# chengzhag/PanFusion

Hardware: AMD Instinct MI355X
Metric: DDIM denoise steps/sec, 512x1024 pano + 20x512^2 views (higher is better)
Workload: dtype fp16; 1 GPU; cfg2: 512x1024 pano + 20x512^2 views, CFG pair, SD-2-base UNet shapes; views=20, cfg_pair=True, hip_graphs=True, parallelism=single

## Files before the change

### include/panfusion_hip.h

```cpp
#ifndef PANFUSION_HIP_H
#define PANFUSION_HIP_H

#include <stddef.h>
#include <stdint.h>

#ifdef __cplusplus
extern "C" {
#endif

typedef enum { PF_OK = 0, PF_ERR_ARG = 1, PF_ERR_LAUNCH = 2, PF_ERR_UNSUPPORTED = 3 } pf_status;
typedef enum { PF_BF16 = 0, PF_F16 = 1, PF_F32 = 2, PF_U8 = 3 } pf_dtype;

int pf_version(void);
const char* pf_last_error_string(void);


pf_status pf_e2p_grid(const double* host_fov, const double* host_theta, const double* host_phi,
                      int ncam, int eh, int ew, int h, int w,
                      float* map_x, float* map_y, float* lonlat, void* stream);

pf_status pf_p2e_grid(const double* host_fov, const double* host_theta, const double* host_phi,
                      int ncam, int ph, int pw, int h, int w,
                      float* map_u, float* map_v, uint8_t* mask, void* stream);

// ... 182 lines not shown
    int M, N, K;
    int dtype; int mode;
} pf_linear_ws_desc;
enum { PF_LWS_16 = 0, PF_LWS_F32 = 1, PF_LWS_GEGLU = 2, PF_LWS_QKV = 3, PF_LWS_F32_LN = 4, PF_LWS_VT = 5 };
int pf_linear_ws_supported(long M, int N, int K, int mode);
pf_status pf_linear_ws(const pf_linear_ws_desc* desc, void* stream);

pf_status pf_conv_in(const float* x, int n, int cin, int h, int w, const float* wgt, const float* bias,
                     int cout, int wrap, int out_dtype, void* y, void* stream);
pf_status pf_conv_out(const void* x, int dtype, int n, int cin, int h, int w, const float* wgt,
                      const float* bias, int cout, int wrap, float* y, void* stream);
pf_status pf_conv_out_gn(const float* x, int n, int cin, int h, int w, const float* scale, const float* shift, int act,
                         const float* wgt_t, const float* bias, int cout, int wrap, float* y, void* stream);

typedef struct {
    const void* q; const void* k; const void* vt; void* out;
    int dtype;
    int B, H, D;
    int nq, nk;
    int q_ld, k_ld, vt_ld, o_ld;
    long q_bs, k_bs, vt_bs, o_bs;
    float scale;
    const float* bias; long bias_ld;
    const uint8_t* flags; int flags_ld;
    float* lse;
    void* workspace; size_t workspace_bytes;
} pf_attn_desc;

pf_status pf_attention(const pf_attn_desc* desc, void* stream);
size_t pf_attention_workspace_size(const pf_attn_desc* desc);

pf_status pf_attention_wide(const pf_attn_desc* desc, void* stream);


pf_status pf_attention_delta(const void* out, const void* dout, int dtype, int B, int H, int D, long nq,
                             int ld, long bs, float* delta, void* stream);

typedef struct {
    const void* q; const void* k; const void* v; const void* dout;
    const void* qt; const void* kt; const void* dot;
    void* dq; void* dk; void* dv;
    int dtype;
    int B, H, D;
    int nq, nk;
    int q_ld, k_ld, v_ld, do_ld;
    int qt_ld, kt_ld, dot_ld;
    int dq_ld, dk_ld, dv_ld;
    long q_bs, k_bs, v_bs, do_bs, qt_bs, kt_bs, dot_bs, dq_bs, dk_bs, dv_bs;
    float scale;
    const float* bias; long bias_ld;
    const uint8_t* flags; int flags_ld;
    const float* lse; const float* delta;
    void* workspace; size_t workspace_bytes;
} pf_attn_bwd_desc;

size_t pf_attention_bwd_workspace_size(const pf_attn_bwd_desc* desc);
pf_status pf_attention_bwd(const pf_attn_bwd_desc* desc, void* stream);

int pf_layernorm_bwd_parts(long rows);
pf_status pf_layernorm_bwd(const void* x, const float* pe, long pe_rows, int dtype, long rows, int C,
                           const float* gamma, float eps, const float* dy, const float* dres, float* dx,
                           float* partials, void* stream);

size_t pf_groupnorm_bwd_workspace_size(int n_img, int hw, int groups);
pf_status pf_groupnorm_bwd(const void* x0, int c0, const void* x1, int c1, int dtype, int n_img, int hw, int groups,
                           float eps, const float* gamma, const float* scale, const float* shift, int act,
// ... 44 lines not shown
```

### panfusion_amd/_lib.py

```python
import ctypes as C
import os

_HERE = os.path.dirname(os.path.abspath(__file__))
LIB_PATH = os.environ.get("PF_HIP_LIB") or os.path.join(_HERE, "libpanfusion_hip.so")

PF_OK = 0
PF_BF16, PF_F16, PF_F32, PF_U8 = 0, 1, 2, 3

c_void_p, c_int, c_long, c_float, c_size_t = C.c_void_p, C.c_int, C.c_long, C.c_float, C.c_size_t
c_dp = C.POINTER(C.c_double)


class ConvDesc(C.Structure):
    _fields_ = [
        ("a0", c_void_p), ("a1", c_void_p), ("c0", c_int), ("c1", c_int),
        ("a0_ld", c_int), ("a1_ld", c_int),
        ("n_img", c_int), ("h_in", c_int), ("w_in", c_int), ("h_out", c_int), ("w_out", c_int),
        ("ksize", c_int), ("stride", c_int), ("pad", c_int), ("upsample", c_int),
        ("w", c_void_p), ("n_out", c_int),
        ("bias", c_void_p), ("rowvec", c_void_p), ("rowvec_ld", c_int),
        ("residual", c_void_p), ("res_ld", c_int), ("res_dtype", c_int),
        ("out", c_void_p), ("out_ld", c_int), ("out_dtype", c_int), ("dtype", c_int),
        ("batch", c_int),
        ("a_bstride", c_long), ("w_bstride", c_long), ("out_bstride", c_long), ("res_bstride", c_long),
# ... 3 lines not shown
        ("a_src_dtype", c_int), ("a_scale", c_void_p), ("a_shift", c_void_p),
    ]


class ConvPlan(C.Structure):
    _fields_ = [
        ("kernel", c_int), ("mrep", c_int), ("nrep", c_int), ("block_rows", c_int), ("waves", c_int), ("ring_slots", c_int),
        ("splits", c_int), ("kb_per_split", c_int), ("m_split", c_int), ("tail_splits", c_int), ("tail_kb", c_int),
        ("gn_rows", c_int), ("n_tickets", c_int), ("workspace_bytes", c_size_t),
    ]


class AttnDesc(C.Structure):
    _fields_ = [
        ("q", c_void_p), ("k", c_void_p), ("vt", c_void_p), ("out", c_void_p),
        ("dtype", c_int), ("B", c_int), ("H", c_int), ("D", c_int), ("nq", c_int), ("nk", c_int),
        ("q_ld", c_int), ("k_ld", c_int), ("vt_ld", c_int), ("o_ld", c_int),
        ("q_bs", c_long), ("k_bs", c_long), ("vt_bs", c_long), ("o_bs", c_long),
        ("scale", c_float),
        ("bias", c_void_p), ("bias_ld", c_long), ("flags", c_void_p), ("flags_ld", c_int),
        ("lse", c_void_p),
        ("workspace", c_void_p), ("workspace_bytes", c_size_t),
    ]


class LinearWsDesc(C.Structure):
    _fields_ = [
        ("a", c_void_p), ("a_ld", c_int), ("w", c_void_p), ("bias", c_void_p),
        ("residual", c_void_p), ("res_ld", c_int), ("out", c_void_p), ("out_ld", c_int),
        ("out_vt", c_void_p), ("vt_ld", c_int), ("rows_per_batch", c_int), ("vt_bs", c_long),
        ("ln_gamma", c_void_p), ("ln_beta", c_void_p), ("ln_eps", c_float), ("ln_out", c_void_p), ("ln_ld", c_int),
        ("M", c_int), ("N", c_int), ("K", c_int), ("dtype", c_int), ("mode", c_int),
    ]


class AttnBwdDesc(C.Structure):
    _fields_ = [
        ("q", c_void_p), ("k", c_void_p), ("v", c_void_p), ("dout", c_void_p),
        ("qt", c_void_p), ("kt", c_void_p), ("dot", c_void_p),
        ("dq", c_void_p), ("dk", c_void_p), ("dv", c_void_p),
        ("dtype", c_int), ("B", c_int), ("H", c_int), ("D", c_int), ("nq", c_int), ("nk", c_int),
        ("q_ld", c_int), ("k_ld", c_int), ("v_ld", c_int), ("do_ld", c_int),
        ("qt_ld", c_int), ("kt_ld", c_int), ("dot_ld", c_int),
        ("dq_ld", c_int), ("dk_ld", c_int), ("dv_ld", c_int),
        ("q_bs", c_long), ("k_bs", c_long), ("v_bs", c_long), ("do_bs", c_long), ("qt_bs", c_long), ("kt_bs", c_long),
        ("dot_bs", c_long), ("dq_bs", c_long), ("dk_bs", c_long), ("dv_bs", c_long),
        ("scale", c_float),
        ("bias", c_void_p), ("bias_ld", c_long), ("flags", c_void_p), ("flags_ld", c_int),
        ("lse", c_void_p), ("delta", c_void_p),
        ("workspace", c_void_p), ("workspace_bytes", c_size_t),
    ]


SIGNATURES = {
    "pf_version": (c_int, []),
    "pf_last_error_string": (C.c_char_p, []),
    "pf_e2p_grid": (c_int, [c_dp, c_dp, c_dp, c_int, c_int, c_int, c_int, c_int,
                            c_void_p, c_void_p, c_void_p, c_void_p]),
    "pf_p2e_grid": (c_int, [c_dp, c_dp, c_dp, c_int, c_int, c_int, c_int, c_int,
                            c_void_p, c_void_p, c_void_p, c_void_p]),
    "pf_py360_e2p": (c_int, [c_void_p, c_int, c_int, c_int, c_int, c_dp, c_dp, c_dp, c_dp, c_dp, c_int, c_int, c_int, c_int,
                             c_void_p, c_void_p]),
    "pf_nearest_indices": (c_int, [c_void_p, c_void_p, c_long, c_int, c_int, c_void_p, c_void_p]),
    "pf_remap": (c_int, [c_void_p, c_int, c_int, c_int, c_int, c_int, c_void_p, c_void_p, c_void_p,
                         c_int, c_int, c_int, c_int, c_void_p, c_void_p]),
    "pf_equi_coords": (c_int, [c_int, c_int, c_void_p, c_void_p]),
# ... 32 lines not shown
                                      c_long, c_int, c_int, c_void_p, c_void_p, c_void_p, c_int, C.c_int64, c_void_p]),
    "pf_cfg_dpmpp_step_pair": (c_int, [c_void_p, c_void_p, c_void_p, c_float, c_float, c_float, c_float, c_float,
                                       c_long, c_int, c_int, c_void_p, c_void_p, c_void_p, c_int, C.c_int64,
                                       c_void_p, c_float, c_void_p, c_void_p]),
    "pf_cfg_inpaint_step_pair": (c_int, [c_void_p, c_void_p, c_void_p, c_float, c_float, c_float, c_float, c_float,
                                         c_long, c_int, c_int, c_void_p, c_void_p, c_void_p, c_int, C.c_int64,
                                         c_void_p, c_float, c_void_p, c_void_p, c_void_p, c_void_p, c_float, c_float,
                                         c_int, c_void_p]),
    "pf_noised_start_pair": (c_int, [c_void_p, c_void_p, c_float, c_float, c_long, c_int, c_int, c_void_p, c_void_p, c_void_p,
                                     c_int, C.c_int64, c_void_p]),
    "pf_upsampled_start_pair": (c_int, [c_void_p, c_void_p, c_float, c_float, c_long, c_int, c_int, c_int, c_int, c_int, c_int,
                                        c_int, c_void_p, c_void_p, c_void_p, c_int, C.c_int64, c_void_p]),
    "pf_conv_gemm":(c_int, [C.POINTER(ConvDesc), c_void_p]),
    "pf_conv_gemm_workspace_size": (c_size_t, [C.POINTER(ConvDesc)]),
    "pf_conv_gemm_gn_rows": (c_int, [C.POINTER(ConvDesc)]),
    "pf_conv_gemm_kernel_id": (c_int, [C.POINTER(ConvDesc)]),
    "pf_conv_gemm_plan": (c_int, [C.POINTER(ConvDesc), c_int, C.POINTER(ConvPlan)]),
    "pf_groupnorm_from_partials": (c_int, [c_void_p, c_int, c_int, c_void_p, c_int, c_int, c_int, c_int, c_int, c_float,
                                           c_void_p, c_void_p, c_void_p, c_void_p, c_void_p]),
    "pf_scale_shift_act_pair": (c_int, [c_void_p, c_int, c_void_p, c_int, c_int, c_int, c_void_p, c_void_p, c_int, c_int,
                                        c_void_p, c_void_p, c_void_p]),
    "pf_debug_gemm_profile": (c_int, [c_void_p, c_long]),
    "pf_linear_ws_supported": (c_int, [c_long, c_int, c_int, c_int]),
    "pf_linear_ws": (c_int, [C.POINTER(LinearWsDesc), c_void_p]),
    "pf_conv_in": (c_int, [c_void_p, c_int, c_int, c_int, c_int, c_void_p, c_void_p, c_int, c_int, c_int,
                           c_void_p, c_void_p]),
    "pf_conv_out": (c_int, [c_void_p, c_int, c_int, c_int, c_int, c_int, c_void_p, c_void_p, c_int, c_int,
                            c_void_p, c_void_p]),
    "pf_conv_out_gn": (c_int, [c_void_p, c_int, c_int, c_int, c_int, c_void_p, c_void_p, c_int, c_void_p, c_void_p, c_int, c_int,
                               c_void_p, c_void_p]),
    "pf_attention": (c_int, [C.POINTER(AttnDesc), c_void_p]),
    "pf_attention_workspace_size": (c_size_t, [C.POINTER(AttnDesc)]),
    "pf_attention_wide": (c_int, [C.POINTER(AttnDesc), c_void_p]),
    "pf_attention_delta": (c_int, [c_void_p, c_void_p, c_int, c_int, c_int, c_int, c_long, c_int, c_long, c_void_p, c_void_p]),
    "pf_attention_bwd": (c_int, [C.POINTER(AttnBwdDesc), c_void_p]),
    "pf_attention_bwd_workspace_size": (c_size_t, [C.POINTER(AttnBwdDesc)]),
    "pf_layernorm_bwd_parts": (c_int, [c_long]),
    "pf_layernorm_bwd": (c_int, [c_void_p, c_void_p, c_long, c_int, c_long, c_int, c_void_p, c_float, c_void_p, c_void_p,
                                 c_void_p, c_void_p, c_void_p]),
    "pf_groupnorm_bwd_workspace_size": (c_size_t, [c_int, c_int, c_int]),
    "pf_groupnorm_bwd": (c_int, [c_void_p, c_int, c_void_p, c_int, c_int, c_int, c_int, c_int, c_float, c_void_p, c_void_p,
                                 c_void_p, c_int, c_void_p, c_void_p, c_void_p, c_void_p, c_void_p, c_size_t, c_void_p]),
    "pf_groupnorm_param_grads_workspace_size": (c_size_t, [c_int, c_int, c_int]),
    "pf_groupnorm_param_grads": (c_int, [c_void_p, c_int, c_void_p, c_int, c_int, c_int, c_int, c_void_p, c_void_p, c_void_p, c_void_p,
                                         c_int, c_void_p, c_void_p, c_void_p, c_size_t, c_void_p]),
    "pf_silu_bwd": (c_int, [c_void_p, c_int, c_void_p, c_long, c_void_p, c_void_p]),
    "pf_im2col3": (c_int, [c_void_p, c_int, c_int, c_int, c_int, c_int, c_int, c_void_p, c_void_p]),
    "pf_lora_fold": (c_int, [c_void_p, c_void_p, c_void_p, c_int, c_int, c_int, c_float, c_int, c_void_p, c_long, c_void_p, c_long,
                             c_void_p, c_long, c_void_p, c_long, c_void_p]),
    "pf_weighted_colsum_workspace_size": (c_size_t, [c_long, c_int, c_int]),
    "pf_weighted_colsum": (c_int, [c_void_p, c_int, c_long, c_int, c_long, c_void_p, c_int, c_long, c_void_p, c_float, c_void_p, c_int,
                                   c_void_p, c_void_p, c_size_t, c_void_p]),
    "pf_zero_insert2": (c_int, [c_void_p, c_int, c_int, c_int, c_int, c_int, c_void_p, c_void_p]),
    "pf_sum2x2": (c_int, [c_void_p, c_int, c_int, c_int, c_int, c_void_p, c_void_p]),
    "pf_pad_width_bwd": (c_int, [c_void_p, c_int, c_int, c_int, c_int, c_int, c_void_p, c_void_p]),
    "pf_crop_width_bwd": (c_int, [c_void_p, c_int, c_int, c_int, c_int, c_int, c_void_p, c_void_p]),
    "pf_transpose_tokens": (c_int, [c_void_p, c_int, c_int, c_long, c_int, c_void_p, c_void_p]),
    "pf_geglu_bwd": (c_int, [c_void_p, c_void_p, c_int, c_long, c_int, c_void_p, c_void_p]),
    "pf_colsum_workspace_size": (c_size_t, [c_long, c_int]),
    "pf_colsum": (c_int, [c_void_p, c_int, c_long, c_int, c_long, c_void_p, c_void_p, c_size_t, c_void_p]),
    "pf_amax_f32": (c_int, [c_void_p, c_long, c_void_p, c_int, c_void_p]),
    "pf_pow2_scale": (c_int, [c_void_p, c_void_p]),
    "pf_scale_f32": (c_int, [c_void_p, c_long, c_void_p, c_int, c_int, c_void_p, c_void_p]),
}


# ... 44 lines not shown
```

### panfusion_amd/engine.py

```python
import os
from types import SimpleNamespace as NS

import torch

from . import ops


def default_precision(dtype):
    env = os.environ.get("PF_PRECISION")
    if env in ("mixed", "fast"):
        return env
    return "mixed" if dtype == torch.float16 else "fast"


RAW_PAIR_FUSED = os.environ.get("PF_RAW_PAIR", "1") != "0"
A32 = os.environ.get("PF_A32", "1") != "0"
TAPING = False
VIRTUAL_PAD = os.environ.get("PF_VIRTUAL_PAD", "1") != "0"
EXACT_UP0 = os.environ.get("PF_EXACT_UP0", "1") != "0"
SUBPIXEL_UP = os.environ.get("PF_SUBPIXEL_UP", "1") != "0"
FUSED_HEAD = os.environ.get("PF_FUSED_HEAD", "1") != "0"


def stream_dtype(dtype, precision):
# ... 400 lines not shown
        y = ops.scale_shift_act(x, skip, n, hw, sc, sh, 1, out_dtype=r.dtype)
    rowvec = temb_all[:, r.temb_off:] if temb_all is not None else None
    wp = w + 2 * wrap
    h1 = ops.conv_gemm(y, r.w1, r.cout, n_img=n, h_in=h, w_in=w, ksize=3, pad=1, bias=r.b1, rowvec=rowvec, gn_stats=True,
                       wrap_pad=wrap, out_dtype=torch.float32 if save is not None else None)
    h1 = ops.carry(h1.view(n, h * wp, r.cout), h1)
    sc, sh = ops.groupnorm_scale_shift(h1, None, n, h * wp, r.norm2.groups, r.norm2.eps, r.norm2.g, r.norm2.b)
    if save is not None:
        save.h1, save.sc2, save.sh2 = h1, sc, sh
    y2 = ops.scale_shift_act(h1, None, n, h * wp, sc, sh, 1, out_dtype=r.dtype)
    if split:
        short = _split_shortcut(r, x, n * hw, max_operand_bytes)
    elif r.ws3 is not None:
        if direct:
            short = exact_gemm_f32(x, r.ws3, r.cout, r.dtype, x1=skip, w_in=n * hw, bias=r.bs, out_dtype=r.stream)
        else:
            if pair is None:
                pair = split_operand(x, skip, dtype=r.dtype)
            short = exact_gemm(pair, r.ws3, r.cout, w_in=n * hw, bias=r.bs, out_dtype=r.stream)
    elif r.ws is not None:
        short = ops.conv_gemm(x, r.ws, r.cout, a1=skip, n_img=n, h_in=h, w_in=w, ksize=1, bias=r.bs)
    else:
        short = x.view(n * hw, r.cout)
    out = ops.conv_gemm(y2, r.w2, r.cout, n_img=n, h_in=h, w_in=wp, ksize=3, pad=1, bias=r.b2, residual=short, gn_stats=True,
                        crop=wrap)
    return ops.carry(out.view(n, h, w, r.cout), out)


def text_kv(a, text):
    n, L = text.shape[:2]
    return ops.linear(text.reshape(n * L, -1), a.wk), ops.linear_t(text, a.wv)


def all_transformers(u):
    for blk in [*u.down, u.mid, *u.up]:
        for t in (blk.attns or []):
            yield t


def self_qkv(a, tokens, n, nk):
    fused = ops.linear_qkv(tokens, a.wqkv, n)
    if fused is not None:
        return fused
    qk = ops.linear(tokens, a.wqk)
    vt = ops.linear_vt(tokens, a.wv, n)
    if vt is None:
        vt = ops.linear_t(tokens.view(n, nk, -1), a.wv)
    return qk, vt


def _attend(a, q_src, kv_tokens, n, nq, nk, head_dim, *, self_attn, residual, kv=None, next_ln=None, split=None):
    Cq = a.dim
    vt = None
    if split is not None and self_attn and n == 1:
        from . import sharding
        o = sharding.split_pano_attention(split, a, q_src, nq)
        if next_ln is not None:
            return ops.linear_ln(o.view(n * nq, Cq), a.wo, a.bo, residual, next_ln.g, next_ln.b, next_ln.eps)
        return ops.linear(o.view(n * nq, Cq), a.wo, bias=a.bo, residual=residual)
    if self_attn:
        qk, vt = self_qkv(a, q_src, n, nk)
        q, k, ld = qk, qk[:, Cq:], 2 * Cq
    else:
        q, ld = ops.linear(q_src, a.wq), Cq
        k = kv[0] if kv is not None else ops.linear(kv_tokens, a.wk)
    if kv is not None:
        vt = kv[1]
    elif vt is None:
        vt = ops.linear_t(kv_tokens.view(n, nk, -1), a.wv)
    o = ops.attention(q, k, vt, n, a.heads, head_dim, nq, nk,
                      q_ld=ld, k_ld=(ld if self_attn else Cq), vt_ld=vt.shape[-1],
                      q_bs=nq * ld, k_bs=nk * (ld if self_attn else Cq), vt_bs=vt.shape[1] * vt.shape[2])
    if next_ln is not None:
        return ops.linear_ln(o.view(n * nq, Cq), a.wo, a.bo, residual, next_ln.g, next_ln.b, next_ln.eps)
    return ops.linear(o.view(n * nq, Cq), a.wo, bias=a.bo, residual=residual)


def run_transformer(t, x, text, kv=None, split=None):
    n, h, w, Cc = x.shape
    hw = h * w
    sc, sh = ops.groupnorm_scale_shift(x, None, n, hw, t.norm.groups, t.norm.eps, t.norm.g, t.norm.b)
    if t.w_in3 is not None:
        tok = exact_gemm_f32(x, t.w_in3, Cc, t.dtype, scale=sc, shift=sh, w_in=n * hw, bias=t.b_in, out_dtype=t.stream)
    else:
        y = ops.scale_shift_act(x, None, n, hw, sc, sh, 0)
        tok = ops.linear(y.view(n * hw, Cc), t.w_in, bias=t.b_in)
    dh = t.attn1.dim // t.attn1.heads
    ln = ops.layernorm(tok, t.ln1.g, t.ln1.b, t.ln1.eps, out_dtype=t.dtype)
    tok, ln = _attend(t.attn1, ln, ln, n, hw, hw, dh, self_attn=True, residual=tok, next_ln=t.ln2, split=split)
    if ln is None:
        ln = ops.layernorm(tok, t.ln2.g, t.ln2.b, t.ln2.eps, out_dtype=t.dtype)
    L = text.shape[1]
    tok, ln = _attend(t.attn2, ln, text.reshape(n * L, -1), n, hw, L, dh, self_attn=False, residual=tok, kv=kv, next_ln=t.ln3)
    if ln is None:
        ln = ops.layernorm(tok, t.ln3.g, t.ln3.b, t.ln3.eps, out_dtype=t.dtype)
    g = ops.linear(ln, t.w_ff1, bias=t.b_ff1, geglu=True)
    if t.w_out3 is not None and os.environ.get("PF_FF2_PAIR", "1") != "0":
        pair = ops.linear(g, t.w_ff2, bias=t.b_ff2, residual=tok, split_out=True)
        out = exact_gemm(pair, t.w_out3, Cc, w_in=n * hw, bias=t.b_out, residual=x.view(n * hw, Cc), gn_stats=True)
    elif t.w_out3 is not None:
        tok = ops.linear(g, t.w_ff2, bias=t.b_ff2, residual=tok)
        out = exact_gemm(split_operand(tok, dtype=t.dtype), t.w_out3, Cc, w_in=n * hw, bias=t.b_out, residual=x.view(n * hw, Cc),
                         gn_stats=True)
    else:
        tok = ops.linear(g, t.w_ff2, bias=t.b_ff2, residual=tok)
        out = ops.linear(tok, t.w_out, bias=t.b_out, residual=x.view(n * hw, Cc), gn_stats=True)
    return ops.carry(out.view(n, h, w, Cc), out)


class Branch:

    def __init__(self, u, latent, timestep, text, pano, pad):
        self.u, self.text, self.pad = u, text, (pano and pad)
        n = latent.shape[0]
        feats = ops.timestep_features(timestep, u.t_dim, u.dtype)
        e = ops.linear(feats, u.w_t1, bias=u.b_t1)
        e = ops.linear(ops.silu(e), u.w_t2, bias=u.b_t2)
        self.temb = ops.linear(ops.silu(e), u.w_temb, bias=u.b_temb, out_dtype=torch.float32)
        self.h = ops.conv_in(latent.float(), u.w_conv_in, u.b_conv_in, u.c0, u.stream, wrap=self.pad)
        self.skips = [self.h]
        self.text_kv = {}
        self.text_ready = None
        self.attn_split = None
        self.attn_help = None
        self.split_streams = None
        self.keep = None

    def precompute_text_kv(self):
        key = (self.text.data_ptr(), self.text._version, tuple(self.text.shape), self.text.dtype, str(self.text.device))
        cache = self.u.__dict__.setdefault("text_kv_cache", {})
        hit = cache.get(key)
        if hit is None:
            if len(cache) >= 4:
                victim = next((ck for ck, h in cache.items() if not h.get("pins")), None)
                if victim is not None:
                    cache.pop(victim)
            hit = {id(t): text_kv(t.attn2, self.text) for t in all_transformers(self.u)}
            hit["text"] = self.text
            cache[key] = hit
        self.text_kv = hit

    def _padded(self, t, p):
        return ops.pad_width(t, p) if (self.pad and t is not None) else t

    def resnet(self, r, skip=False, save=None):
        s = self.skips.pop() if skip else None
        if self.pad and VIRTUAL_PAD:
            self.h = run_resnet(r, self.h, s, self.temb, wrap=2, save=save)
        elif self.pad:
            out = run_resnet(r, self._padded(self.h, 2), self._padded(s, 2), self.temb, save=save)
            self.h = ops.crop_width(out, 2)
        else:
            self.h = run_resnet(r, self.h, s, self.temb, save=save)

    def attention(self, t):
        if self.text_ready is not None:
            torch.cuda.current_stream(self.h.device).wait_event(self.text_ready)
            self.text_ready = None
        split = None
        if self.attn_split is not None:
            from . import sharding
            if sharding.splits_pano_attention(self.attn_split, self.h.shape[1] * self.h.shape[2]) and self.h.shape[0] == 1:
                split = self.attn_split
        if split is not None and self.split_streams is not None:
            main, side = self.split_streams
            main.wait_stream(side)
            x_in = self.h
            with torch.cuda.stream(main):
                self.h = run_transformer(t, x_in, self.text, self.text_kv.get(id(t)), split=split)
            side.wait_stream(main)
            if self.keep is not None:
                self.keep.extend((x_in, self.h))
        else:
            self.h = run_transformer(t, self.h, self.text, self.text_kv.get(id(t)), split=split)
        if self.attn_help is not None:
            self.attn_help(t, self.h)

    def push(self):
        self.skips.append(self.h)

    def downsample(self, d):
        virt = self.pad and VIRTUAL_PAD
        x = self.h if virt else self._padded(self.h, 2)
        n, h, w, Cc = x.shape
        geo = dict(wrap_pad=2, crop=1) if virt else {}
        if d.w3 is not None:
            y = exact_gemm(split_operand(x, dtype=self.u.dtype), d.w3, d.c, n_img=n, h_in=h, w_in=w, ksize=3, stride=2,
                           pad=1, bias=d.b, out_dtype=self.u.stream, **geo)
        else:
            y = ops.conv_gemm(x, d.w, d.c, n_img=n, h_in=h, w_in=w, ksize=3, stride=2, pad=1, bias=d.b, **geo)
        if virt:
            self.h = y.view(n, (h - 1) // 2 + 1, y.shape[0] // (n * ((h - 1) // 2 + 1)), d.c)
            return
        y = y.view(n, (h - 1) // 2 + 1, (w - 1) // 2 + 1, d.c)
        self.h = ops.crop_width(y, 1) if self.pad else y

    def upsample(self, up):
        virt = self.pad and VIRTUAL_PAD
        if getattr(up, "w4s", None) is not None and (virt or not self.pad) and self.h.dtype == torch.float32:
            n, h, w, Cc = self.h.shape
            y = exact_gemm(split_operand(self.h, dtype=self.u.dtype), up.w4s, up.c, n_img=n, h_in=h, w_in=w, ksize=3, pad=1, upsample=1,
                           bias=up.b, out_dtype=self.u.stream, gn_stats=not self.pad, subpixel=True, **(dict(wrap_pad=1, crop=2) if virt else {}))
            self.h = y.view(n, 2 * h, 2 * w, up.c) if virt else ops.carry(y.view(n, 2 * h, 2 * w, up.c), y)
            return
        x = to16(self.h if virt else self._padded(self.h, 1), self.u.dtype)
        n, h, w, Cc = x.shape
        geo = dict(wrap_pad=1, crop=2) if virt else {}
# ... 214 lines not shown
```

### panfusion_amd/models/pano/MVGenModel.py

```python
import contextlib
import os

import torch
import torch.nn as nn

from ... import engine
from .modules import WarpAttn, camera_groups


def _repack_hook(module, incompatible):
    module.repack()


class MultiViewBaseModel(nn.Module):
    def __init__(self, unet, pano_unet, pers_cn=None, pano_cn=None, pano_pad=True,
                 compute_dtype=torch.float16, precision=None, differentiable=False):
        super().__init__()
        self.differentiable = differentiable
        self.precision = precision or engine.default_precision(compute_dtype)
        self.unet = unet
        self.pano_unet = pano_unet
        self.pers_cn = pers_cn
        self.pano_cn = pano_cn
        self.pano_pad = pano_pad
# ... 108 lines not shown
        tensors = self.trainable_tensors()
        return tuple((id(t), t._version) for t in tensors[self._n_epa:self._n_lora_epa])

    def forward(self, latents, pano_latent, timestep, prompt_embd, pano_prompt_embd, cameras,
                pers_layout_cond=None, pano_layout_cond=None):
        args = (latents, pano_latent, timestep, prompt_embd, pano_prompt_embd, cameras, pers_layout_cond, pano_layout_cond)
        if self.differentiable and torch.is_grad_enabled():
            from ... import train_engine
            params = [t for t in self.trainable_tensors() if t.requires_grad]
            if params:
                out = train_engine.DenoiserFunction.apply(self, args, *params)
                return out if isinstance(out, tuple) else (None, out)
        return self._forward(*args)

    @torch.no_grad()
    def refold_lora(self):
        if not self._packed:
            return
        key = self._lora_versions()
        for (which, *_), u in self._packed.items():
            if which.endswith("_cn") or getattr(u, "lora_key", key) == key:
                continue
            for t in engine.all_transformers(u):
                engine.fold_attention(t.attn1)
                engine.fold_attention(t.attn2)
            cache = getattr(u, "text_kv_cache", {})
            for ck in [ck for ck, hit in cache.items() if not hit.get("pins")]:
                del cache[ck]
            for hit in cache.values():
                for t in engine.all_transformers(u):
                    k, vt = engine.text_kv(t.attn2, hit["text"])
                    hit[id(t)][0].copy_(k)
                    hit[id(t)][1].copy_(vt)
            u.lora_key = key

    @torch.no_grad()
    def _forward(self, latents, pano_latent, timestep, prompt_embd, pano_prompt_embd, cameras,
                 pers_layout_cond=None, pano_layout_cond=None, tape=None):
        self.refold_lora()
        if self.pers_cn is None:
            pers_layout_cond = None
        if self.pano_cn is None:
            pano_layout_cond = None
        dev = pano_latent.device
        dt = self.compute_dtype
        two = self.unet is not None
        branches = []
        cn_res = {}
        shard = getattr(self, "shard", None)
        from ... import train_engine
        if tape is not None:
            if shard is not None:
                raise NotImplementedError("the training path covers the un-sharded denoiser")
            from ... import train_engine
            make_branch = lambda *a, **k: train_engine.TrainBranch(tape, *a, **k)
        else:
            make_branch = engine.Branch
        cn_recs = {}

        def controlnet(which, br, latent, t, cond):
            c = self.packed(which, dev)
            if tape is not None and any(p_.requires_grad for p_ in getattr(self, which).parameters()):
                cn_res[id(br)], cn_recs[id(br)] = train_engine.controlnet_forward(c, latent, t, br.text, cond)
            else:
                cn_res[id(br)] = engine.run_controlnet(c, latent, t, br.text, cond)
        if two:
# ... 194 lines not shown
```

### panfusion_amd/ops.py

```python
import ctypes as C
import os

import numpy as np
import torch

from . import _lib
from ._lib import PF_BF16, PF_F16, PF_F32, AttnBwdDesc, AttnDesc, ConvDesc, ConvPlan, LinearWsDesc, check

_DT = {torch.bfloat16: PF_BF16, torch.float16: PF_F16, torch.float32: PF_F32}

TRACE = None


class _PlanCache(__import__("threading").local):
    LIMIT = 4096

    def __init__(self):
        self.plans = {}


_PLANS = _PlanCache()
SPLITK_INKERNEL = os.environ.get("PF_SPLITK_INKERNEL") == "1"


# ... 747 lines not shown
                                    _p(out), _stream()), "pf_conv_out_gn")
    return out


def attention(q, k, vt, B, H, D, nq, nk, *, q_ld, k_ld, vt_ld, o_ld=None, q_bs, k_bs, vt_bs, o_bs=None,
              scale=None, bias=None, flags=None, out=None, lse=None):
    o_ld = o_ld or H * D
    o_bs = o_bs if o_bs is not None else nq * o_ld
    if out is None:
        out = torch.empty(B, nq, o_ld, device=q.device, dtype=q.dtype)
    d = AttnDesc()
    d.q, d.k, d.vt, d.out = _p(q), _p(k), _p(vt), _p(out)
    d.dtype, d.B, d.H, d.D, d.nq, d.nk = dt(q), B, H, D, nq, nk
    d.q_ld, d.k_ld, d.vt_ld, d.o_ld = q_ld, k_ld, vt_ld, o_ld
    d.q_bs, d.k_bs, d.vt_bs, d.o_bs = q_bs, k_bs, vt_bs, o_bs
    d.scale = scale if scale is not None else D ** -0.5
    d.bias, d.bias_ld = _p(bias), (_ld(bias) if bias is not None else 0)
    d.flags, d.flags_ld = _p(flags), (_ld(flags) if flags is not None else 0)
    d.lse = _p(lse)
    d.workspace, d.workspace_bytes = None, 0
    if bias is not None and lse is None:
        nbytes = _lib.lib().pf_attention_workspace_size(C.byref(d))
        if nbytes:
            ws = torch.empty(nbytes, device=q.device, dtype=torch.uint8)
            d.workspace, d.workspace_bytes = _p(ws), nbytes
    _traced("k_attention", 4.0 * B * H * nq * nk * D,
            lambda: check(_lib.lib().pf_attention(C.byref(d), _stream()), "pf_attention"),
            "B%d H%d D%d nq%d nk%d bias%d" % (B, H, D, nq, nk, bias is not None))
    return out


WIDE_HEAD_DIMS = (128, 256, 512)


def attention_wide(q, k, vt, B, H, D, nq, nk, *, q_ld, k_ld, vt_ld, o_ld=None, q_bs, k_bs, vt_bs, o_bs=None, scale=None, out=None):
    o_ld = o_ld or H * D
    o_bs = o_bs if o_bs is not None else nq * o_ld
    if out is None:
        out = torch.empty(B, nq, o_ld, device=q.device, dtype=q.dtype)
    d = AttnDesc()
    d.q, d.k, d.vt, d.out = _p(q), _p(k), _p(vt), _p(out)
    d.dtype, d.B, d.H, d.D, d.nq, d.nk = dt(q), B, H, D, nq, nk
    d.q_ld, d.k_ld, d.vt_ld, d.o_ld = q_ld, k_ld, vt_ld, o_ld
    d.q_bs, d.k_bs, d.vt_bs, d.o_bs = q_bs, k_bs, vt_bs, o_bs
    d.scale = scale if scale is not None else D ** -0.5
    d.bias, d.bias_ld, d.flags, d.flags_ld, d.lse = None, 0, None, 0, None
    d.workspace, d.workspace_bytes = None, 0
    _traced("k_attention_wide", 4.0 * B * H * nq * nk * D,
            lambda: check(_lib.lib().pf_attention_wide(C.byref(d), _stream()), "pf_attention_wide"),
            "B%d H%d D%d nq%d nk%d" % (B, H, D, nq, nk))
    return out


def transpose_tokens(x, out=None):
    B, T, Cc = x.shape
    if out is None:
        out = torch.empty(B, Cc, T, device=x.device, dtype=x.dtype)
    if x.dtype == torch.float32:
        check(_lib.lib().pf_nhwc_to_nchw(_p(x), dt(x), B, Cc, 1, T, dt(out), _p(out), _stream()), "pf_nhwc_to_nchw")
    else:
        check(_lib.lib().pf_transpose_tokens(_p(x), dt(x), B, T, Cc, _p(out), _stream()), "pf_transpose_tokens")
    return out


def attention_delta(out, dout, B, H, D, nq):
    delta = torch.empty(B, H, nq, device=out.device, dtype=torch.float32)
# ... 176 lines not shown
```

Baseline: 17.24 steps/s.

## Fold Q/O projections into cached text K/V and fuse cross-attention with residual LayerNorm

Result: no change. 17.36 steps/s, median of 6 (+0.7%).

```diff
diff --git a/include/panfusion_hip.h b/include/panfusion_hip.h
--- a/include/panfusion_hip.h
+++ b/include/panfusion_hip.h
@@ -238,6 +238,25 @@
 
 pf_status pf_attention_wide(const pf_attn_desc* desc, void* stream);
 
+#define PF_TEXT_ATTN_C 320
+#define PF_TEXT_ATTN_H 5
+#define PF_TEXT_ATTN_KP 96
+#define PF_TEXT_ATTN_MK_LD 328
+#define PF_TEXT_ATTN_NVT_LD 104
+typedef struct {
+    const void* x; int x_ld;
+    const void* mk; const void* nvt;
+    const float* bias_o;
+    const float* residual; int res_ld;
+    float* out; int out_ld;
+    const float* ln_gamma; const float* ln_beta; float ln_eps; void* ln_out; int ln_ld;
+    int B, H, D, C;
+    int nq, nk, kp;
+    int dtype;
+} pf_text_attn_desc;
+int pf_text_attention_fused_supported(int dtype, int B, int H, int D, int C, int nq, int nk);
+pf_status pf_text_attention_fused(const pf_text_attn_desc* desc, void* stream);
+
 
 pf_status pf_attention_delta(const void* out, const void* dout, int dtype, int B, int H, int D, long nq,
                              int ld, long bs, float* delta, void* stream);
diff --git a/panfusion_amd/_lib.py b/panfusion_amd/_lib.py
--- a/panfusion_amd/_lib.py
+++ b/panfusion_amd/_lib.py
@@ -59,6 +59,19 @@
         ("ln_gamma", c_void_p), ("ln_beta", c_void_p), ("ln_eps", c_float), ("ln_out", c_void_p), ("ln_ld", c_int),
         ("M", c_int), ("N", c_int), ("K", c_int), ("dtype", c_int), ("mode", c_int),
     ]
+
+
+class TextAttnDesc(C.Structure):
+    _fields_ = [
+        ("x", c_void_p), ("x_ld", c_int), ("mk", c_void_p), ("nvt", c_void_p), ("bias_o", c_void_p),
+        ("residual", c_void_p), ("res_ld", c_int), ("out", c_void_p), ("out_ld", c_int),
+        ("ln_gamma", c_void_p), ("ln_beta", c_void_p), ("ln_eps", c_float), ("ln_out", c_void_p), ("ln_ld", c_int),
+        ("B", c_int), ("H", c_int), ("D", c_int), ("C", c_int), ("nq", c_int), ("nk", c_int), ("kp", c_int),
+        ("dtype", c_int),
+    ]
+
+
+TEXT_ATTN_C, TEXT_ATTN_H, TEXT_ATTN_KP, TEXT_ATTN_MK_LD, TEXT_ATTN_NVT_LD = 320, 5, 96, 328, 104
 
 
 class AttnBwdDesc(C.Structure):
@@ -157,6 +170,8 @@
     "pf_attention": (c_int, [C.POINTER(AttnDesc), c_void_p]),
     "pf_attention_workspace_size": (c_size_t, [C.POINTER(AttnDesc)]),
     "pf_attention_wide": (c_int, [C.POINTER(AttnDesc), c_void_p]),
+    "pf_text_attention_fused_supported": (c_int, [c_int, c_int, c_int, c_int, c_int, c_int, c_int]),
+    "pf_text_attention_fused": (c_int, [C.POINTER(TextAttnDesc), c_void_p]),
     "pf_attention_delta": (c_int, [c_void_p, c_void_p, c_int, c_int, c_int, c_int, c_long, c_int, c_long, c_void_p, c_void_p]),
     "pf_attention_bwd": (c_int, [C.POINTER(AttnBwdDesc), c_void_p]),
     "pf_attention_bwd_workspace_size": (c_size_t, [C.POINTER(AttnBwdDesc)]),
diff --git a/panfusion_amd/csrc/pf_text_attention.hip b/panfusion_amd/csrc/pf_text_attention.hip
--- /dev/null
+++ b/panfusion_amd/csrc/pf_text_attention.hip
@@ -0,0 +1,338 @@
+#include "pf_common.h"
+#include <atomic>
+
+namespace pf {
+namespace {
+
+constexpr int TA_C = PF_TEXT_ATTN_C, TA_H = PF_TEXT_ATTN_H, TA_KP = PF_TEXT_ATTN_KP;
+constexpr int TA_MK_LD = PF_TEXT_ATTN_MK_LD, TA_NV_LD = PF_TEXT_ATTN_NVT_LD;
+constexpr int TA_MK_BYTES = TA_KP * TA_MK_LD * 2;
+constexpr int TA_NV_BYTES = TA_C * TA_NV_LD * 2;
+constexpr int TA_MK_PIECES = (TA_MK_BYTES + 1023) / 1024;
+constexpr int TA_NV_PIECES = (TA_NV_BYTES + 1023) / 1024;
+constexpr int TA_MK_LDS = TA_MK_PIECES * 1024, TA_NV_LDS = TA_NV_PIECES * 1024;
+constexpr int TA_STG_LD = 36;
+constexpr int TA_STG_BYTES = 32 * TA_STG_LD * 4;
+constexpr int TA_SMEM = TA_MK_LDS + TA_NV_LDS + 4 * TA_STG_BYTES;
+static_assert(TA_C == 320 && TA_KP == 96 && TA_KP % 32 == 0, "the kernel is written for 10 channel blocks and 3 key tiles");
+static_assert((TA_MK_LD / 8) % 2 == 1 && (TA_NV_LD / 8) % 2 == 1, "an odd number of 16-byte chunks per row keeps the fragment reads conflict free");
+static_assert(2 * 32 * TA_MK_LD * 2 + 20 * 32 < 65536 && 9 * 32 * TA_NV_LD * 2 + 6 * 32 < 65536, "fragment offsets are ds_read immediates");
+
+struct TaParams {
+    const unsigned short* x;
+    const unsigned short* mk;
+    const unsigned short* nvt;
+    const float* bias;
+    const float* residual;
+    float* out;
+    const float* g;
+    const float* b;
+    unsigned short* ln_out;
+    float eps;
+    int x_ld, res_ld, out_ld, ln_ld;
+    int nq, nk, xcd_map;
+};
+
+template <typename T>
+__global__ __launch_bounds__(256, 1) void k_text_attention_fused(const TaParams p) {
+    extern __shared__ __attribute__((aligned(16))) unsigned char smem[];
+    typedef typename Mfma32<T>::frag frag;
+    const int t = threadIdx.x, lane = t & 63;
+    const int wave = __builtin_amdgcn_readfirstlane(t >> 6);
+    const int ql = lane & 31, hi = lane >> 5;
+    const int nqb = p.nq >> 7;
+    int b, qb;
+    if (p.xcd_map) {
+        const int xcd = blockIdx.x & 7, idx = blockIdx.x >> 3;
+        b = xcd + 8 * (idx / nqb);
+        qb = idx - (idx / nqb) * nqb;
+    } else {
+        b = blockIdx.x / nqb;
+        qb = blockIdx.x - b * nqb;
+    }
+    b = __builtin_amdgcn_readfirstlane(b);
+    const long row0 = static_cast<long>(b) * p.nq + qb * 128 + wave * 32;
+
+    unsigned char* mkS = smem;
+    unsigned char* nvS = smem + TA_MK_LDS;
+    float* stg = reinterpret_cast<float*>(smem + TA_MK_LDS + TA_NV_LDS + wave * TA_STG_BYTES);
+
+    auto uniform_ptr = [](const unsigned short* ptr) __attribute__((always_inline)) {
+        const unsigned long long v = reinterpret_cast<unsigned long long>(ptr);
+        const unsigned lo = __builtin_amdgcn_readfirstlane(static_cast<unsigned>(v));
+        const unsigned hi_ = __builtin_amdgcn_readfirstlane(static_cast<unsigned>(v >> 32));
+        return reinterpret_cast<unsigned short*>(static_cast<unsigned long long>(lo) | (static_cast<unsigned long long>(hi_) << 32));
+    };
+    auto dma_image = [&](const unsigned short* src, auto bytes_tag, unsigned char* dst) __attribute__((always_inline)) {
+        constexpr int BYTES = decltype(bytes_tag)::value, PIECES = (BYTES + 1023) / 1024;
+        const __amdgpu_buffer_rsrc_t rs = __builtin_amdgcn_make_buffer_rsrc(uniform_ptr(src), 0, BYTES, 0x00020000);
+#pragma unroll
+        for (int j = 0; j < (PIECES + 3) / 4; ++j) {
+            const int piece = 4 * j + 3 < PIECES ? wave + 4 * j : min(wave + 4 * j, PIECES - 1);
+            __builtin_amdgcn_raw_ptr_buffer_load_lds(rs, (__attribute__((address_space(3))) void*)(dst + piece * 1024), 16,
+                                                     static_cast<unsigned>(lane * 16), piece * 1024, 0, 0);
+        }
+    };
+    const std::integral_constant<int, TA_MK_BYTES> MKB;
+    const std::integral_constant<int, TA_NV_BYTES> NVB;
+    const unsigned short* mk_b = p.mk + static_cast<long>(b) * TA_H * (TA_MK_BYTES / 2);
+    const unsigned short* nv_b = p.nvt + static_cast<long>(b) * TA_H * (TA_NV_BYTES / 2);
+
+    dma_image(mk_b, MKB, mkS);
+
+    frag xf[20];
+    {
+        const unsigned short* xp = p.x + (row0 + ql) * p.x_ld + 8 * hi;
+#pragma unroll
+        for (int ks = 0; ks < 20; ++ks) xf[ks] = __builtin_bit_cast(frag, *reinterpret_cast<const u16x8*>(xp + 16 * ks));
+    }
+
+    f32x16 acc[10];
+#pragma unroll
+    for (int d = 0; d < 10; ++d)
+#pragma unroll
+        for (int r = 0; r < 16; ++r) acc[d][r] = 0.f;
+
+    const unsigned char* mrow = mkS + ql * (TA_MK_LD * 2) + hi * 16;
+    const unsigned char* nrow = nvS + ql * (TA_NV_LD * 2) + hi * 16;
+
+    const int c4 = lane & 7, rr = lane >> 3;
+    float4 val[10][4];
+
+    auto load_residual = [&](int d0, int d1) __attribute__((always_inline)) {
+#pragma unroll
+        for (int d = d0; d < d1; ++d)
+#pragma unroll
+            for (int i = 0; i < 4; ++i)
+                val[d][i] = *reinterpret_cast<const float4*>(p.residual + (row0 + 8 * i + rr) * p.res_ld + d * 32 + 4 * c4);
+    };
+    constexpr int TA_RES_EARLY = 6;
+
+    auto head = [&](int h, auto last_tag) __attribute__((always_inline)) {
+        constexpr bool LAST = decltype(last_tag)::value;
+        asm volatile("s_waitcnt vmcnt(0)" ::: "memory");
+        __syncthreads();
+#ifdef PF_TA_ABL_NODMA
+        if (h == 0)
+#endif
+        dma_image(nv_b + static_cast<long>(h) * (TA_NV_BYTES / 2), NVB, nvS);
+
+        f32x16 s[3];
+#pragma unroll
+        for (int tt = 0; tt < 3; ++tt)
+#pragma unroll
+            for (int r = 0; r < 16; ++r) s[tt][r] = 0.f;
+        {
+            u16x8 af[3][3];
+            auto rd = [&](int ks) __attribute__((always_inline)) {
+#pragma unroll
+                for (int tt = 0; tt < 3; ++tt) af[ks % 3][tt] = *reinterpret_cast<const u16x8*>(mrow + tt * 32 * (TA_MK_LD * 2) + ks * 32);
+            };
+            rd(0);
+            rd(1);
+#pragma unroll
+            for (int ks = 0; ks < 20; ++ks) {
+                if (ks + 2 < 20) rd(ks + 2);
+                __builtin_amdgcn_sched_barrier(0);
+#pragma unroll
+                for (int tt = 0; tt < 3; ++tt) s[tt] = Mfma32<T>::run(__builtin_bit_cast(frag, af[ks % 3][tt]), xf[ks], s[tt]);
+                __builtin_amdgcn_sched_barrier(0);
+            }
+        }
+
+        float m = -INFINITY;
+#pragma unroll
+        for (int tt = 0; tt < 3; ++tt)
+#pragma unroll
+            for (int r = 0; r < 16; ++r) {
+                const int key = 32 * tt + (r & 3) + 8 * (r >> 2) + 4 * hi;
+                if (key >= p.nk) s[tt][r] = -INFINITY;
+                m = fmaxf(m, s[tt][r]);
+            }
+        {
+            float a_ = m, b_ = m;
+            asm volatile("s_nop 1\n\tv_permlane32_swap_b32 %0, %1\n\ts_nop 1" : "+v"(a_), "+v"(b_));
+            m = fmaxf(a_, b_);
+        }
+        float l = 0.f;
+#pragma unroll
+        for (int tt = 0; tt < 3; ++tt)
+#pragma unroll
+            for (int r = 0; r < 16; ++r) {
+                s[tt][r] = __builtin_amdgcn_exp2f(s[tt][r] - m);
+                l += s[tt][r];
+            }
+        {
+            float a_ = l, b_ = l;
+            asm volatile("s_nop 1\n\tv_permlane32_swap_b32 %0, %1\n\ts_nop 1" : "+v"(a_), "+v"(b_));
+            l = a_ + b_;
+        }
+        const float inv = 1.0f / l;
+        frag pb[6];
+#pragma unroll
+        for (int kk = 0; kk < 6; ++kk) {
+            u16x8 v;
+#pragma unroll
+            for (int e = 0; e < 8; ++e) v[e] = from_f32<T>(s[kk >> 1][8 * (kk & 1) + e] * inv);
+            pb[kk] = __builtin_bit_cast(frag, v);
+        }
+
+        asm volatile("s_waitcnt vmcnt(0)" ::: "memory");
+        __syncthreads();
+#ifndef PF_TA_ABL_NODMA
+        if constexpr (!LAST) dma_image(mk_b + static_cast<long>(h + 1) * (TA_MK_BYTES / 2), MKB, mkS);
+#endif
+        if constexpr (LAST) {
+#ifndef PF_TA_ABL_NOEPI
+            load_residual(0, TA_RES_EARLY);
+#endif
+        }
+
+        {
+            u16x8 nf[3][5];
+            auto rd = [&](int gi) __attribute__((always_inline)) {
+#pragma unroll
+                for (int e = 0; e < 5; ++e)
+                    nf[gi % 3][e] = *reinterpret_cast<const u16x8*>(nrow + (5 * (gi & 1) + e) * 32 * (TA_NV_LD * 2) + (gi >> 1) * 32);
+            };
+            rd(0);
+            rd(1);
+#pragma unroll
+            for (int gi = 0; gi < 12; ++gi) {
+                if (gi + 2 < 12) rd(gi + 2);
+                __builtin_amdgcn_sched_barrier(0);
+#pragma unroll
+                for (int e = 0; e < 5; ++e)
+                    acc[5 * (gi & 1) + e] = Mfma32<T>::run(__builtin_bit_cast(frag, nf[gi % 3][e]), pb[gi >> 1], acc[5 * (gi & 1) + e]);
+                __builtin_amdgcn_sched_barrier(0);
+            }
+        }
+    };
+#pragma unroll 1
+    for (int h = 0; h < TA_H - 1; ++h) head(h, std::false_type());
+    head(TA_H - 1, std::true_type());
+
+#ifdef PF_TA_ABL_NOEPI
+    {
+        float a_ = 0.f;
+#pragma unroll
+        for (int d = 0; d < 10; ++d)
+#pragma unroll
+            for (int r = 0; r < 16; ++r) a_ += acc[d][r];
+        if (a_ == 123.456f) p.out[row0] = a_;
+        return;
+    }
+#endif
+    load_residual(TA_RES_EARLY, 10);
+    float sum[4] = {0.f, 0.f, 0.f, 0.f};
+#pragma unroll
+    for (int d = 0; d < 10; ++d) {
+#pragma unroll
+        for (int g4 = 0; g4 < 4; ++g4)
+            *reinterpret_cast<float4*>(stg + ql * TA_STG_LD + 8 * g4 + 4 * hi) =
+                float4{acc[d][4 * g4], acc[d][4 * g4 + 1], acc[d][4 * g4 + 2], acc[d][4 * g4 + 3]};
+        __builtin_amdgcn_wave_barrier();
+        const float4 bo = *reinterpret_cast<const float4*>(p.bias + d * 32 + 4 * c4);
+#pragma unroll
+        for (int i = 0; i < 4; ++i) {
+            const long row = row0 + 8 * i + rr;
+            const float4 o = *reinterpret_cast<const float4*>(stg + (8 * i + rr) * TA_STG_LD + 4 * c4);
+            const float4 res = val[d][i];
+            float4 v;
+            v.x = (o.x + bo.x) + res.x;
+            v.y = (o.y + bo.y) + res.y;
+            v.z = (o.z + bo.z) + res.z;
+            v.w = (o.w + bo.w) + res.w;
+            *reinterpret_cast<float4*>(p.out + row * p.out_ld + d * 32 + 4 * c4) = v;
+            val[d][i] = v;
+            sum[i] += (v.x + v.y) + (v.z + v.w);
+        }
+        __builtin_amdgcn_wave_barrier();
+    }
+    float mean[4], rstd[4];
+#pragma unroll
+    for (int i = 0; i < 4; ++i) {
+        float sm = sum[i];
+        sm += __shfl_xor(sm, 1);
+        sm += __shfl_xor(sm, 2);
+        sm += __shfl_xor(sm, 4);
+        mean[i] = sm * (1.0f / TA_C);
+        float q = 0.f;
+#pragma unroll
+        for (int d = 0; d < 10; ++d) {
+            const float a0 = val[d][i].x - mean[i], a1 = val[d][i].y - mean[i], a2 = val[d][i].z - mean[i], a3 = val[d][i].w - mean[i];
+            q += (a0 * a0 + a1 * a1) + (a2 * a2 + a3 * a3);
+        }
+        q += __shfl_xor(q, 1);
+        q += __shfl_xor(q, 2);
+        q += __shfl_xor(q, 4);
+        rstd[i] = rsqrtf(q * (1.0f / TA_C) + p.eps);
+    }
+#pragma unroll
+    for (int d = 0; d < 10; ++d) {
+        const float4 gg = *reinterpret_cast<const float4*>(p.g + d * 32 + 4 * c4);
+        const float4 bb = *reinterpret_cast<const float4*>(p.b + d * 32 + 4 * c4);
+#pragma unroll
+        for (int i = 0; i < 4; ++i) {
+            const long row = row0 + 8 * i + rr;
+            u16x4 w;
+            w[0] = from_f32<T>((val[d][i].x - mean[i]) * rstd[i] * gg.x + bb.x);
+            w[1] = from_f32<T>((val[d][i].y - mean[i]) * rstd[i] * gg.y + bb.y);
+            w[2] = from_f32<T>((val[d][i].z - mean[i]) * rstd[i] * gg.z + bb.z);
+            w[3] = from_f32<T>((val[d][i].w - mean[i]) * rstd[i] * gg.w + bb.w);
+            *reinterpret_cast<u16x4*>(p.ln_out + row * p.ln_ld + d * 32 + 4 * c4) = w;
+        }
+    }
+}
+
+template <typename T>
+pf_status ta_launch(const TaParams& p, int blocks, hipStream_t st) {
+    static std::atomic<unsigned long long> attr_devs{0};
+    int dev = 0;
+    (void)hipGetDevice(&dev);
+    const unsigned long long bit = 1ULL << (dev & 63);
+    if (!(attr_devs.load(std::memory_order_acquire) & bit)) {
+        const hipError_t e = hipFuncSetAttribute(reinterpret_cast<const void*>(k_text_attention_fused<T>), hipFuncAttributeMaxDynamicSharedMemorySize, TA_SMEM);
+        PF_REQUIRE(e == hipSuccess, "pf_text_attention_fused: the device does not grant %d bytes of LDS per workgroup (%s)", TA_SMEM, hipGetErrorString(e));
+        attr_devs.fetch_or(bit, std::memory_order_release);
+    }
+    hipLaunchKernelGGL((k_text_attention_fused<T>), dim3(blocks), dim3(256), TA_SMEM, st, p);
+    PF_CHECK_LAUNCH("pf_text_attention_fused");
+    return PF_OK;
+}
+
+}
+}
+
+extern "C" int pf_text_attention_fused_supported(int dtype, int B, int H, int D, int C, int nq, int nk) {
+    return (dtype == PF_BF16 || dtype == PF_F16) && C == PF_TEXT_ATTN_C && H == PF_TEXT_ATTN_H && D * H == C && B > 0 && nq > 0 && nq % 128 == 0 &&
+           nk >= 1 && nk <= PF_TEXT_ATTN_KP && static_cast<long>(B) * (nq / 128) < (1L << 31);
+}
+
+extern "C" pf_status pf_text_attention_fused(const pf_text_attn_desc* d, void* stream) {
+    using namespace pf;
+    PF_REQUIRE(d != nullptr, "pf_text_attention_fused: null descriptor");
+    if (!pf_text_attention_fused_supported(d->dtype, d->B, d->H, d->D, d->C, d->nq, d->nk)) {
+        set_error("pf_text_attention_fused: serves C == 320, H == 5, D == 64, 1 <= nk <= %d, nq a multiple of 128, fp16 / bf16 (got dtype %d B %d H %d D %d C %d nq %d nk %d)",
+                  PF_TEXT_ATTN_KP, d->dtype, d->B, d->H, d->D, d->C, d->nq, d->nk);
+        return PF_ERR_UNSUPPORTED;
+    }
+    PF_REQUIRE(d->x && d->mk && d->nvt && d->bias_o && d->residual && d->out && d->ln_gamma && d->ln_beta && d->ln_out, "pf_text_attention_fused: null operand");
+    PF_REQUIRE(aligned16(d->x) && aligned16(d->mk) && aligned16(d->nvt) && aligned16(d->bias_o) && aligned16(d->residual) && aligned16(d->out) &&
+               aligned16(d->ln_gamma) && aligned16(d->ln_beta) && aligned16(d->ln_out), "pf_text_attention_fused: operands must be 16-byte aligned");
+    PF_REQUIRE(d->kp == PF_TEXT_ATTN_KP, "pf_text_attention_fused: mk / nvt must be padded to %d key slots (got %d)", PF_TEXT_ATTN_KP, d->kp);
+    PF_REQUIRE(d->x_ld >= d->C && d->x_ld % 8 == 0 && d->ln_ld >= d->C && d->ln_ld % 8 == 0, "pf_text_attention_fused: x_ld / ln_ld must hold 320 columns in 16-byte chunks");
+    PF_REQUIRE(d->res_ld >= d->C && d->res_ld % 4 == 0 && d->out_ld >= d->C && d->out_ld % 4 == 0, "pf_text_attention_fused: res_ld / out_ld must hold 320 fp32 columns in 16-byte chunks");
+    PF_REQUIRE(d->ln_eps > 0.f, "pf_text_attention_fused: ln_eps must be positive");
+    TaParams p;
+    p.x = static_cast<const unsigned short*>(d->x);
+    p.mk = static_cast<const unsigned short*>(d->mk);
+    p.nvt = static_cast<const unsigned short*>(d->nvt);
+    p.bias = d->bias_o; p.residual = d->residual; p.out = d->out;
+    p.g = d->ln_gamma; p.b = d->ln_beta; p.ln_out = static_cast<unsigned short*>(d->ln_out); p.eps = d->ln_eps;
+    p.x_ld = d->x_ld; p.res_ld = d->res_ld; p.out_ld = d->out_ld; p.ln_ld = d->ln_ld;
+    p.nq = d->nq; p.nk = d->nk; p.xcd_map = (d->B % 8 == 0) ? 1 : 0;
+    const int blocks = d->B * (d->nq / 128);
+    PF_DISPATCH_16(d->dtype, "pf_text_attention_fused", return (ta_launch<T>(p, blocks, as_stream(stream))));
+    return PF_OK;
+}
diff --git a/panfusion_amd/engine.py b/panfusion_amd/engine.py
--- a/panfusion_amd/engine.py
+++ b/panfusion_amd/engine.py
@@ -456,6 +456,15 @@
     return ops.linear(text.reshape(n * L, -1), a.wk), ops.linear_t(text, a.wv)
 
 
+def text_fold(a, text, kv, out=None):
+    n, L = text.shape[:2]
+    D = a.dim // a.heads
+    serves = getattr(ops, "text_attention_fused_serves", None)
+    if serves is None or a.bo is None or not serves(a.wq.dtype, n, a.heads, D, a.dim, 128, L):
+        return None
+    return ops.fold_text_operands(kv[0], kv[1], a.wq, a.wo, n, a.heads, D, L, out=out)
+
+
 def all_transformers(u):
     for blk in [*u.down, u.mid, *u.up]:
         for t in (blk.attns or []):
@@ -500,7 +509,7 @@
     return ops.linear(o.view(n * nq, Cq), a.wo, bias=a.bo, residual=residual)
 
 
-def run_transformer(t, x, text, kv=None, split=None):
+def run_transformer(t, x, text, kv=None, split=None, fold=None):
     n, h, w, Cc = x.shape
     hw = h * w
     sc, sh = ops.groupnorm_scale_shift(x, None, n, hw, t.norm.groups, t.norm.eps, t.norm.g, t.norm.b)
@@ -515,7 +524,10 @@
     if ln is None:
         ln = ops.layernorm(tok, t.ln2.g, t.ln2.b, t.ln2.eps, out_dtype=t.dtype)
     L = text.shape[1]
-    tok, ln = _attend(t.attn2, ln, text.reshape(n * L, -1), n, hw, L, dh, self_attn=False, residual=tok, kv=kv, next_ln=t.ln3)
+    if fold is not None and not TAPING and ops.text_attention_fused_ok(ln, tok, n, t.attn2.heads, dh, hw, L):
+        tok, ln = ops.text_attention_fused(ln, fold[0], fold[1], t.attn2.bo, tok, t.ln3.g, t.ln3.b, t.ln3.eps, n, t.attn2.heads, dh, hw, L)
+    else:
+        tok, ln = _attend(t.attn2, ln, text.reshape(n * L, -1), n, hw, L, dh, self_attn=False, residual=tok, kv=kv, next_ln=t.ln3)
     if ln is None:
         ln = ops.layernorm(tok, t.ln3.g, t.ln3.b, t.ln3.eps, out_dtype=t.dtype)
     g = ops.linear(ln, t.w_ff1, bias=t.b_ff1, geglu=True)
@@ -560,6 +572,10 @@
                 if victim is not None:
                     cache.pop(victim)
             hit = {id(t): text_kv(t.attn2, self.text) for t in all_transformers(self.u)}
+            for t in all_transformers(self.u):
+                fold = text_fold(t.attn2, self.text, hit[id(t)])
+                if fold is not None:
+                    hit[("fold", id(t))] = fold
             hit["text"] = self.text
             cache[key] = hit
         self.text_kv = hit
@@ -591,12 +607,12 @@
             main.wait_stream(side)
             x_in = self.h
             with torch.cuda.stream(main):
-                self.h = run_transformer(t, x_in, self.text, self.text_kv.get(id(t)), split=split)
+                self.h = run_transformer(t, x_in, self.text, self.text_kv.get(id(t)), split=split, fold=self.text_kv.get(("fold", id(t))))
             side.wait_stream(main)
             if self.keep is not None:
                 self.keep.extend((x_in, self.h))
         else:
-            self.h = run_transformer(t, self.h, self.text, self.text_kv.get(id(t)), split=split)
+            self.h = run_transformer(t, self.h, self.text, self.text_kv.get(id(t)), split=split, fold=self.text_kv.get(("fold", id(t))))
         if self.attn_help is not None:
             self.attn_help(t, self.h)
 
diff --git a/panfusion_amd/models/pano/MVGenModel.py b/panfusion_amd/models/pano/MVGenModel.py
--- a/panfusion_amd/models/pano/MVGenModel.py
+++ b/panfusion_amd/models/pano/MVGenModel.py
@@ -164,6 +164,9 @@
                     k, vt = engine.text_kv(t.attn2, hit["text"])
                     hit[id(t)][0].copy_(k)
                     hit[id(t)][1].copy_(vt)
+                    fold = hit.get(("fold", id(t)))
+                    if fold is not None:
+                        engine.text_fold(t.attn2, hit["text"], hit[id(t)], out=fold)
             u.lora_key = key
 
     @torch.no_grad()
diff --git a/panfusion_amd/ops.py b/panfusion_amd/ops.py
--- a/panfusion_amd/ops.py
+++ b/panfusion_amd/ops.py
@@ -803,6 +803,60 @@
 
 WIDE_HEAD_DIMS = (128, 256, 512)
 
+TEXT_FUSED = os.environ.get("PF_TEXT_FUSED", "1") != "0"
+
+
+def text_attention_fused_serves(dtype, B, H, D, C, nq, nk):
+    if not TEXT_FUSED or dtype not in (torch.float16, torch.bfloat16):
+        return False
+    return bool(_lib.lib().pf_text_attention_fused_supported(_DT[dtype], B, H, D, C, nq, nk))
+
+
+def text_attention_fused_ok(x, residual, B, H, D, nq, nk):
+    if x.dim() != 2 or x.stride(-1) != 1 or x.stride(0) % 8 or x.shape[0] != B * nq:
+        return False
+    if residual is None or residual.dtype != torch.float32 or residual.dim() != 2 or residual.stride(-1) != 1 or residual.stride(0) % 4:
+        return False
+    return text_attention_fused_serves(x.dtype, B, H, D, x.shape[1], nq, nk)
+
+
+def fold_text_operands(k, vt, wq, wo, B, H, D, nk, scale=None, out=None):
+    Cc = H * D
+    KP, MK_LD, NV_LD = _lib.TEXT_ATTN_KP, _lib.TEXT_ATTN_MK_LD, _lib.TEXT_ATTN_NVT_LD
+    c2 = (scale if scale is not None else D ** -0.5) * 1.4426950408889634
+    k32 = k.float().view(B, nk, H, D).permute(0, 2, 1, 3)
+    v32 = vt[:, :, :nk].float().reshape(B, H, D, nk)
+    wq32 = wq.float().view(H, D, Cc)
+    wo32 = wo.float().view(Cc, H, D).permute(1, 0, 2)
+    mk = torch.zeros(B, H, KP, MK_LD, device=k.device, dtype=torch.float32)
+    mk[:, :, :nk, :Cc] = torch.matmul(k32, wq32.unsqueeze(0)) * c2
+    nv = torch.zeros(B, H, Cc, KP, device=k.device, dtype=torch.float32)
+    nv[:, :, :, :nk] = torch.matmul(wo32.unsqueeze(0), v32)
+    j = torch.arange(KP, device=k.device)
+    key_of_slot = (j & ~12) | ((j & 8) >> 1) | ((j & 4) << 1)
+    nvt = torch.zeros(B, H, Cc, NV_LD, device=k.device, dtype=torch.float32)
+    nvt[..., :KP] = nv[..., key_of_slot]
+    if out is not None:
+        out[0].copy_(mk)
+        out[1].copy_(nvt)
+        return out
+    return mk.to(k.dtype), nvt.to(k.dtype)
+
+
+def text_attention_fused(x, mk, nvt, bias_o, residual, gamma, beta, eps, B, H, D, nq, nk):
+    rows, Cc = x.shape
+    out = torch.empty(rows, Cc, device=x.device, dtype=torch.float32)
+    ln_out = torch.empty(rows, Cc, device=x.device, dtype=x.dtype)
+    d = _lib.TextAttnDesc()
+    d.x, d.x_ld, d.mk, d.nvt, d.bias_o = _p(x), _ld(x), _p(mk), _p(nvt), _p(bias_o)
+    d.residual, d.res_ld, d.out, d.out_ld = _p(residual), _ld(residual), _p(out), Cc
+    d.ln_gamma, d.ln_beta, d.ln_eps, d.ln_out, d.ln_ld = _p(gamma), _p(beta), float(eps), _p(ln_out), Cc
+    d.B, d.H, d.D, d.C, d.nq, d.nk, d.kp, d.dtype = B, H, D, Cc, nq, nk, mk.shape[2], dt(x)
+    _traced("k_text_attention_fused", 4.0 * rows * Cc * Cc + 4.0 * B * H * nq * nk * D,
+            lambda: check(_lib.lib().pf_text_attention_fused(C.byref(d), _stream()), "pf_text_attention_fused"),
+            "B%d H%d D%d nq%d nk%d" % (B, H, D, nq, nk))
+    return out, ln_out
+
 
 def attention_wide(q, k, vt, B, H, D, nq, nk, *, q_ld, k_ld, vt_ld, o_ld=None, q_bs, k_bs, vt_bs, o_bs=None, scale=None, out=None):
     o_ld = o_ld or H * D
```
